# horizon-research/Fov-3DGS

Measured on AMD Instinct MI355X. Metric: frames/sec at 1080p foveated (bicycle-scale), higher is better.
Workload: dtype f32; 1 GPU; S-6M bicycle-scale cloud, 4-layer foveated render (fov_pcheck_obb), the reference's 9 fixed gazes (0.25 i, 0.25 j) in turn, one camera per GPU; gaussians=6000000, width=1920, height=1080, sh_degree=3, model_layout=the reference's tensor interface (render(packed=None)), overlap_successive_frames=True, parallelism=views1

## Files before the change

### fov-3dgs_amd/csrc/common.h

```cpp
#pragma once
#include <hip/hip_runtime.h>
#include <stdint.h>
#include <stddef.h>
#include "../../include/fovraster.h"

#define FR_TILE 16
#define FR_TILE_PIX 256
#define FR_FOV_LEVELS 4
#define FR_FOV_MAX_LEVELS 8
#define FR_SORT_LDS_MAX 8192
#ifndef FR_BIN_THREADS
#define FR_BIN_THREADS 768
#endif
#define FR_BIN_BLOCKS 512
#define FR_PROJ_MAX_WAVES 8192
#define FR_CROW_PAD (64 * FR_PROJ_MAX_WAVES)
#define FR_LDS_HIST_MAX_TILES 16384
#define FR_ITEM_NONE 0xffffffffu
#define FR_LDS_HIST16_MAX_TILES 34816
#define FR_HIST16_MAX_SLABS (65535 / FR_BIN_THREADS)
#define FR_BIG_TNUM 64
#define FR_GIANT_TNUM 1024
#define FR_GIANT_MAX 64
#define FR_SORT_SPLIT_MIN 16384
#define FR_SORT_CHUNK_TARGET 960
#define FR_SORT_FINE_BUCKETS 2048
#define FR_SORT_MAX_CHUNKS(D) ((size_t)(D) / FR_SORT_CHUNK_TARGET + (size_t)(D) / FR_SORT_SPLIT_MIN + 16)
#define FR_LV_BBOX_STRIDE 32
#define FR_SLAB_CTR_WORDS 32

namespace fr {

#define FR_VARIANT_SUM_NOSTATS 100
#define FR_VARIANT_FOV8 101
__host__ __device__ inline bool has_stats(int v) { return v == FR_VARIANT_PCHECK_OBB_SUM || v == FR_VARIANT_PCHECK_OBB_MAX || v == FR_VARIANT_PCHECK_OBB_LWMC; }
__host__ __device__ inline bool has_backward(int v) { return v == FR_VARIANT_ORIGINAL || has_stats(v); }
__host__ __device__ constexpr inline bool is_fov(int v) { return v == FR_VARIANT_FOV_PCHECK_OBB || v == FR_VARIANT_FOV8 || v == FR_VARIANT_NAIVE_FOV_PCHECK_OBB || v == FR_VARIANT_MMFR_PCHECK_OBB; }
// ... 289 lines not shown
{
	const bwd_u2 r = __builtin_amdgcn_permlane16_swap(__float_as_uint(a), __float_as_uint(b), false, false);
	return __uint_as_float(r.x) + __uint_as_float(r.y);
}
__device__ __forceinline__ float row_sum16(float x)
{
	x += __builtin_bit_cast(float, __builtin_amdgcn_update_dpp(0, __builtin_bit_cast(int, x), 0xB1, 0xF, 0xF, false));
	x += __builtin_bit_cast(float, __builtin_amdgcn_update_dpp(0, __builtin_bit_cast(int, x), 0x4E, 0xF, 0xF, false));
	x += __builtin_bit_cast(float, __builtin_amdgcn_update_dpp(0, __builtin_bit_cast(int, x), 0x141, 0xF, 0xF, false));
	x += __builtin_bit_cast(float, __builtin_amdgcn_update_dpp(0, __builtin_bit_cast(int, x), 0x140, 0xF, 0xF, false));
	return x;
}

__device__ __forceinline__ float act_scale(float raw) { return expf(raw); }
__device__ __forceinline__ float act_opacity(float raw) { return 1.0f / (1.0f + expf(-raw)); }
__device__ __forceinline__ float4 act_rotation(float4 v, float *inv_norm = nullptr)
{
	const float n = sqrtf(v.x * v.x + v.y * v.y + v.z * v.z + v.w * v.w);
	const float d = fmaxf(n, 1e-12f);
	if (inv_norm) *inv_norm = n > 1e-12f ? 1.0f / n : -1e12f;
	return make_float4(v.x / d, v.y / d, v.z / d, v.w / d);
}

struct FwdCtx {
	fr_forward_args *a;
	hipStream_t stream;
	int gx, gy, T;
	int fov_split;
	uint8_t *visibility;
	int bin_wgs;
	int hist_mode;
	int scan_fused;
	int heavy4, heavy2;
	int heavy8;
	int heavy16, heavy32;
	int n_items;
	int proj_waves, proj_cpw;
	int64_t capacity;
	int64_t items_cap;
	uint32_t *totals_host_dev;
	uint32_t totals_seq;
	float focal_x, focal_y;
	FovParams fov;
	GeomWS geom;
	ImageWS img;
	BinWS bin;
};
struct AuxStream { int device = -1; hipStream_t main = nullptr, s, s2; hipEvent_t fork, fork2, join, join2; bool ok = false; };
AuxStream *aux_stream(hipStream_t main);
int launch_tile_levels(FwdCtx &c);
int launch_pad_levels(FwdCtx &c);
int launch_pack_geom(int P, const float *means3D, const float *scales, const float *rotations, const float *opacities, int levels,
	const float *highest_levels, float *out, hipStream_t stream);
// ... 34 lines not shown
```

### fov-3dgs_amd/csrc/preprocess.hip

```cpp
#include "common.h"
#include "tile_scan.h"
#include <cstdlib>

namespace fr {

struct M3 { float c[3][3]; };
__device__ __forceinline__ M3 m3_cols(float a0, float a1, float a2, float b0, float b1, float b2, float c0, float c1, float c2)
{
	M3 m; m.c[0][0] = a0; m.c[0][1] = a1; m.c[0][2] = a2; m.c[1][0] = b0; m.c[1][1] = b1; m.c[1][2] = b2;
	m.c[2][0] = c0; m.c[2][1] = c1; m.c[2][2] = c2; return m;
}
__device__ __forceinline__ M3 m3_mul(const M3 &a, const M3 &b)
{
	M3 r;
#pragma unroll
	for (int col = 0; col < 3; col++)
#pragma unroll
		for (int row = 0; row < 3; row++)
			r.c[col][row] = a.c[0][row] * b.c[col][0] + a.c[1][row] * b.c[col][1] + a.c[2][row] * b.c[col][2];
	return r;
}
__device__ __forceinline__ M3 m3_t(const M3 &a)
{
	M3 r;
// ... 828 lines not shown
			const float dch[12] = { dh0.x, dh0.y, dh0.z, dh0.w, dh1.x, dh1.y, dh1.z, dh1.w, dh2.x, dh2.y, dh2.z, dh2.w };
			const float oh[4] = { oph.x, oph.y, oph.z, oph.w };
#pragma unroll
			for (int l = FR_FOV_LEVELS; l < NLV; l++)
			{
				if (l >= lo && l <= hi)
				{
					const int m = l - FR_FOV_LEVELS;
					float4 v;
					v.x = fmaxf(FR_SH_C0 * dch[3 * m] + rest[0], 0.0f);
					v.y = fmaxf(FR_SH_C0 * dch[3 * m + 1] + rest[1], 0.0f);
					v.z = fmaxf(FR_SH_C0 * dch[3 * m + 2] + rest[2], 0.0f);
					v.w = oh[m];
					lv[l] = v;
				}
			}
		}
	}
}

#define BUMP_TILE(ti) do { if (LDSH == 2) atomicAdd(&lds_hist[(ti) >> 1], 1u << (16 * ((ti) & 1))); \
	else if (LDSH) atomicAdd(&lds_hist[(ti)], 1u); else atomicAdd(&a.tile_count[(ti)], 1u); } while (0)
static_assert((FR_BIN_THREADS / 64) * FR_HIST16_MAX_SLABS * 64 <= 65535, "a workgroup's items must fit a 16-bit tile count (LDSH == 2)");
template <int VARIANT, int LDSH, bool PACKED = false, bool CROW = false>
__global__ void __launch_bounds__(FR_BIN_THREADS) k_bin(const PreArgs a)
{
	static_assert(!(PACKED && CROW), "the packed model layout has its own rows");
	constexpr bool CULL = VARIANT != FR_VARIANT_ORIGINAL;
	constexpr bool FOV = is_fov(VARIANT);
	constexpr bool LEVELCOL = is_levelcol(VARIANT);
	constexpr int NLV = level_rows(VARIANT);
	constexpr uint32_t LV_MASK = (1u << NLV) - 1u, LV_BLEND = 1u << NLV;
	static_assert(!(PACKED && FOV && !LEVELCOL), "the shared-model foveated variant has no packed layout");
		extern __shared__ __attribute__((aligned(16))) uint32_t lds_hist[];
	const int lane = threadIdx.x & 63;
	const int hist_words = LDSH == 2 ? (a.T + 1) / 2 : (LDSH ? a.T : 0);
	uint32_t *lds_tab = lds_hist + hist_words;
	const int tab_words = (a.T + 7) / 8;
	const bool ldst = FOV && a.lds_tiles && a.geom.slab_ctr[3] == 0u;
	if (FOV && a.lds_tiles)
	{
		const float *gmin = a.tile_lv + a.T, *gbl = a.tile_lv + 4 * (size_t)a.T;
		for (int t0 = threadIdx.x; t0 < a.T; t0 += 16 * FR_BIN_THREADS)
		{
			float v[16], f[16];
#pragma unroll
			for (int k = 0; k < 16; k++) { const int t = min(t0 + k * FR_BIN_THREADS, a.T - 1); v[k] = gmin[t]; f[k] = gbl[t]; }
#pragma unroll
			for (int k = 0; k < 16; k++)
			{
				const int t = t0 + k * FR_BIN_THREADS;
				uint32_t nib = t < a.T ? ((v[k] == v[k] ? (uint32_t)min(max(f2i(v[k]), 0), 7) : 7u) | (f[k] != 0.0f ? 8u : 0u)) : 0u;
				nib <<= 4 * (lane & 7);
				nib |= (uint32_t)__shfl_xor((int)nib, 1); nib |= (uint32_t)__shfl_xor((int)nib, 2); nib |= (uint32_t)__shfl_xor((int)nib, 4);
				if ((lane & 7) == 0 && (t >> 3) < tab_words) lds_tab[t >> 3] = nib;
			}
		}
	}
	if (LDSH)
		for (int t = threadIdx.x; t < hist_words; t += FR_BIN_THREADS) lds_hist[t] = 0;
	__shared__ int s_gitem[FR_GIANT_MAX];
	__shared__ uint32_t s_gcount[FR_GIANT_MAX], s_gmask[FR_GIANT_MAX];
	__shared__ uint32_t s_ng;
	__shared__ uint4 s_lvbox[5];
	if (FOV && threadIdx.x < 5) s_lvbox[threadIdx.x] = *(const uint4 *)(a.lv_bbox + threadIdx.x * FR_LV_BBOX_STRIDE);
	if (threadIdx.x < FR_GIANT_MAX) { s_gcount[threadIdx.x] = 0; s_gmask[threadIdx.x] = 0; }
	__shared__ uint32_t s_next_slab;
	if (threadIdx.x == 0) { s_ng = 0; s_next_slab = 0; }
	__syncthreads();
#define TILE_FILTER(ti, olim, pass_out, bits_out) do { \
		if (ldst) { const uint32_t nb_ = (lds_tab[(ti) >> 3] >> (4 * ((ti) & 7))) & 15u; \
			pass_out = (float)(nb_ & 7u) < (olim); bits_out = (1u << min(nb_ & 7u, 3u)) | (((nb_ & 8u) >> 3) << NLV); } \
		else { const float lv_ = tile_min[(ti)]; pass_out = lv_ < (olim); \
			bits_out = pass_out ? ((1u << min(max(f2i(lv_), 0), NLV - 1)) | (tile_bl[(ti)] != 0.0f ? LV_BLEND : 0u)) : 0u; } } while (0)
	float4 *const s_orec = (float4 *)(lds_hist + ((hist_words + ((FOV && a.lds_tiles) ? tab_words : 0) + 3) & ~3));
	int *const s_own = (int *)(s_orec + 4 * FR_BIN_THREADS);
	const uint32_t *const s_wbase = (const uint32_t *)(s_own + FR_BIN_THREADS);
	const uint32_t *const g_wbase = a.geom.wbase;
	if (a.wbase_lds)
	{
		uint32_t *const dst = (uint32_t *)(s_own + FR_BIN_THREADS);
		for (int w0 = threadIdx.x; w0 <= a.proj_waves; w0 += 16 * FR_BIN_THREADS)
		{
			uint32_t v[16];
#pragma unroll
			for (int k = 0; k < 16; k++) v[k] = a.geom.wbase[min(w0 + k * FR_BIN_THREADS, a.proj_waves)];
#pragma unroll
			for (int k = 0; k < 16; k++) if (w0 + k * FR_BIN_THREADS <= a.proj_waves) dst[w0 + k * FR_BIN_THREADS] = v[k];
		}
		__syncthreads();
	}
	float cam_vm[16], cam_pm[16];
	{
#pragma unroll
		for (int i = 0; i < 16; i++)
		{
			cam_vm[i] = __builtin_bit_cast(float, __builtin_amdgcn_readfirstlane(__builtin_bit_cast(int, a.viewmatrix[i])));
			cam_pm[i] = __builtin_bit_cast(float, __builtin_amdgcn_readfirstlane(__builtin_bit_cast(int, a.projmatrix[i])));
		}
	}
	const int V = (int)a.geom.slab_ctr[1];
	const int nslabs = (V + 63) / 64;
	const int nwaves = (int)gridDim.x * (FR_BIN_THREADS / 64);
	const float *tile_min = FOV ? a.tile_lv + a.T : nullptr;
	const float *tile_bl = FOV ? a.tile_lv + 4 * (size_t)a.T : nullptr;
	auto walk_uniform = [&](const int ox0, const int oy0, const int ow, const uint32_t on, const Obb &ob, const float olim,
		const uint32_t k0, const uint32_t kstep, uint32_t &cnt, uint32_t &bits) __attribute__((always_inline))
	{
		const float rw = 1.0f / (float)ow;
		for (uint32_t k = k0; k < on; k += kstep)
		{
			const uint32_t j = k + lane;
			const bool valid = j < on;
			int ry = (int)(((float)j + 0.5f) * rw);
			int rx = (int)j - ry * ow;
			if (rx < 0) { ry--; rx += ow; } else if (rx >= ow) { ry++; rx -= ow; }
			const int x = ox0 + rx, y = oy0 + ry;
			const int ti = valid ? y * a.gx + x : 0;
			bool pass = valid;
			uint32_t m = 0;
			if (CULL)
			{
				uint32_t lb = 0;
				if (FOV) { bool lp; TILE_FILTER(ti, olim, lp, lb); pass = pass && lp; }
				pass = pass && obb_hits_tile(ob, x, y);
				if (FOV && pass) m = lb;
// ... 12 lines not shown
	{
		const int lo_bit = __ffs((int)(lvmask & LV_MASK)) - 1, hi_bit = 31 - __clz((int)(lvmask & LV_MASK));
		lowest = fminf(lowest, (float)lo_bit);
		highest = fmaxf(highest, (float)hi_bit);
		be_blend = (lvmask & LV_BLEND) != 0;
	};
	auto range_word = [&](const uint32_t count, const float lowest, const float highest, const bool be_blend) __attribute__((always_inline))
	{
		if (count == 0) return FR_ITEM_NONE;
		if (!FOV) return 0u;
		const int lo = f2i(lowest);
		int hi = f2i(highest);
		if (be_blend) hi = min(hi + 1, a.levels - 1);
		return (uint32_t)(lo & 0xff) | ((uint32_t)(hi & 0xff) << 8);
	};
	float4 *const orec = s_orec + 4 * (threadIdx.x & ~63);
	const bool rows_ok = a.colors_precomp == nullptr &&
		(PACKED || (LEVELCOL ? a.M * 3 >= 45 : (a.shs_rest != nullptr ? (a.M - 1) * 3 >= 45 : a.M * 3 >= 48)));
	for (;;)
	{
	uint32_t q_ = 0;
	if (lane == 0) q_ = atomicAdd(&s_next_slab, 1u);
	q_ = (uint32_t)__builtin_amdgcn_readfirstlane((int)q_);
	constexpr int BW_ = FR_BIN_THREADS / 64;
	const int slab = (int)blockIdx.x * BW_ + (int)(q_ % BW_) + (int)(q_ / BW_) * nwaves;
	if (slab >= nslabs) break;
	const int nv = min(64, V - slab * 64);
	const int item = slab * 64 + lane;
	float4 wr[4];
	float3 fpos = make_float3(0.f, 0.f, 0.f), fconic = make_float3(0.f, 0.f, 0.f);
	{
		RawGaussian g;
		g.p[0] = g.p[1] = g.p[2] = 0.f; g.sc[0] = g.sc[1] = g.sc[2] = 0.f; g.q = make_float4(0, 0, 0, 0); g.hl = 0.f;
		int gidx = 0;
		const bool valid = item < V;
		if (valid)
		{
			auto slot_in = [&](const uint32_t *wb) -> uint32_t {
				int lo = 0, hi = a.proj_waves;
				const uint32_t first = (uint32_t)slab * 64u;
				while (hi - lo > 1) { const int mid = (lo + hi) >> 1; if (wb[mid] <= first) lo = mid; else hi = mid; }
				int w = lo;
				while ((uint32_t)item >= wb[w + 1]) w++;
				return (uint32_t)w * (uint32_t)a.proj_cpw * 64u + ((uint32_t)item - wb[w]);
			};
			const uint32_t slot = a.wbase_lds ? slot_in(s_wbase) : slot_in(g_wbase);
			if (CROW)
// ... 167 lines not shown
#pragma unroll
		for (int l = 0; l < NLV; l++) lv[l] = make_float4(0, 0, 0, 0);
		if (lr != FR_ITEM_NONE) colour_item<VARIANT, PACKED>(a, rows_ok, lr, r, lv);
		if constexpr (LEVELCOL && NLV == FR_FOV_LEVELS) rows_store<4>(lv, orec, a.geom.lvl + 4 * (size_t)slab * 64, nv, lane);
		else if constexpr (LEVELCOL)
		{
			const float4 lo4[4] = { lv[0], lv[1], lv[2], lv[3] }, hi4[4] = { lv[4], lv[5], lv[6], lv[7] };
			rows_store<4>(lo4, orec, a.geom.lvl + 4 * (size_t)slab * 64, nv, lane);
			rows_store<4>(hi4, orec, a.geom.lvl_hi + 4 * (size_t)slab * 64, nv, lane);
		}
		else rows_store<3>(r, orec, a.geom.rec + 3 * (size_t)slab * 64, nv, lane);
	}
	}
	__syncthreads();
	const int ng = min((int)s_ng, FR_GIANT_MAX);
	for (int g = 0; g < ng; g++)
	{
		const float4 *wr = a.geom.wrec + 4 * (size_t)s_gitem[g];
		const float4 w0 = wr[0], w1 = wr[1], w2 = wr[2], w3 = wr[3];
		const Obb ob = make_obb(w0.x, w0.y, make_float4(w0.z, w0.w, w1.x, w1.y), make_float2(w1.z, w1.w));
		const uint32_t xy = __float_as_uint(w2.z);
		uint32_t cnt = 0, bits = 0;
		walk_uniform((int)(xy & 0xffffu), (int)(xy >> 16), (int)__float_as_uint(w2.w), __float_as_uint(w3.x), ob, w3.y + 1,
			(uint32_t)(threadIdx.x & ~63u), (uint32_t)FR_BIN_THREADS, cnt, bits);
		if (lane == 0) { atomicAdd(&s_gcount[g], cnt); if (FOV) atomicOr(&s_gmask[g], bits); }
	}
	__syncthreads();
	if ((int)threadIdx.x < ng)
	{
		const int gitem = s_gitem[threadIdx.x];
		const uint32_t gcount = s_gcount[threadIdx.x];
		const float4 w2 = a.geom.wrec[4 * (size_t)gitem + 2], w3 = a.geom.wrec[4 * (size_t)gitem + 3];
		float lowest = w3.y, highest = 0.0f;
		bool be_blend = false;
		if (FOV && gcount != 0) range_from_mask(s_gmask[threadIdx.x], lowest, highest, be_blend);
		const uint32_t lr = range_word(gcount, lowest, highest, be_blend);
		a.geom.lrange[gitem] = lr;
		if (gcount == 0)
		{
			const uint32_t gi = __float_as_uint(w2.x) & 0x3fffffffu;
			a.radii[gi] = 0;
			if (a.visibility) a.visibility[gi] = 0;
		}
		else
		{
			float4 r[3], lv[NLV];
#pragma unroll
			for (int i = 0; i < 3; i++) r[i] = a.geom.rec[3 * (size_t)gitem + i];
#pragma unroll
			for (int l = 0; l < NLV; l++) lv[l] = make_float4(0, 0, 0, 0);
			colour_item<VARIANT, PACKED>(a, rows_ok, lr, r, lv);
			if (LEVELCOL)
			{
#pragma unroll
				for (int l = 0; l < NLV; l++)
					(l < FR_FOV_LEVELS ? a.geom.lvl : a.geom.lvl_hi)[(size_t)gitem * FR_FOV_LEVELS + (l & 3)] = lv[l];
			}
			else { a.geom.rec[3 * (size_t)gitem + 1] = r[1]; a.geom.rec[3 * (size_t)gitem + 2] = r[2]; }
		}
	}
	if (LDSH)
	{
		__syncthreads();
		uint32_t *out = a.hist + (size_t)blockIdx.x * a.T;
		for (int t0 = threadIdx.x; t0 < a.T; t0 += 4 * FR_BIN_THREADS)
		{
			uint32_t h[4], o[4];
#pragma unroll
			for (int k = 0; k < 4; k++)
			{
				const int t = t0 + k * FR_BIN_THREADS;
				h[k] = t < a.T ? (LDSH == 2 ? (lds_hist[t >> 1] >> (16 * (t & 1))) & 0xffffu : lds_hist[t]) : 0u;
			}
#pragma unroll
			for (int k = 0; k < 4; k++) o[k] = h[k] ? atomicAdd(&a.tile_count[t0 + k * FR_BIN_THREADS], h[k]) : 0u;
#pragma unroll
			for (int k = 0; k < 4; k++) { const int t = t0 + k * FR_BIN_THREADS; if (t < a.T && h[k]) out[t] = o[k]; }
		}
		if (LDSH == 1 && a.fuse_scan)
		{
			__shared__ uint32_t s_last_wg;
			__syncthreads();
			if (threadIdx.x == 0) s_last_wg = atomicAdd(a.geom.slab_ctr + 4, 1u) == gridDim.x - 1 ? 1u : 0u;
			__syncthreads();
			if (!s_last_wg || threadIdx.x >= FR_TILE_SCAN_THREADS) return;
			tile_scan_body<FR_TILE_SCAN_THREADS, true>(a.ts, lds_hist);
		}
	}
}
#undef BUMP_TILE
#undef TILE_FILTER

struct EmitArgs {
	int P, gx, gy, T;
	const int *radii;
	GeomWS geom;
	const float *highest_levels;
	const float *tile_lv;
	const uint32_t *lv_bbox;
	int lds_tiles;
	const uint2 *ranges;
	uint32_t *cursor;
	uint64_t *entries;
	const uint32_t *hist;
	const uint32_t *totals;
	uint32_t capacity;
	uint32_t items_cap;
};
#ifndef FR_EMIT_THREADS
#define FR_EMIT_THREADS FR_BIN_THREADS
#endif
#define NEXT_SLOT(ti) (LDSH == 2 ? a.ranges[(ti)].x + pre_row[(ti)] + ((atomicAdd(&lds_cur[(ti) >> 1], 1u << (16 * ((ti) & 1))) >> (16 * ((ti) & 1))) & 0xffffu) \
	: LDSH ? atomicAdd(&lds_cur[(ti)], 1u) : a.ranges[(ti)].x + atomicAdd(&a.cursor[(ti)], 1u))
template <int VARIANT, int LDSH>
__global__ void __launch_bounds__(FR_EMIT_THREADS) k_emit(const EmitArgs a)
{
	constexpr bool CULL = VARIANT != FR_VARIANT_ORIGINAL;
	constexpr bool FOV = VARIANT == FR_VARIANT_FOV_PCHECK_OBB;
	extern __shared__ __attribute__((aligned(16))) uint32_t lds_cur[];
#ifdef FR_EMIT_TIMERS
	const uint64_t tm_entry = wall_clock64(); uint64_t tm_pro = 0, tm_loop = 0, tm_walk = 0, tm_big = 0, tm_drain = 0, tm_pre = 0, tm_mid = 0, tm_ta = 0; int tm_slabs = 0, tm_steps = 0;
#endif
	if (a.totals[0] > a.capacity || a.totals[5] > a.items_cap) return;
	const int lane = threadIdx.x & 63;
	const int cur_words = LDSH == 2 ? (a.T + 1) / 2 : (LDSH ? a.T : 0);
	const uint32_t *const pre_row = a.hist + (LDSH ? (size_t)blockIdx.x * a.T : 0);
	uint32_t *lds_tab = lds_cur + cur_words;
	const int tab_words = (a.T + 7) / 8;
	const bool ldst = FOV && a.lds_tiles && a.geom.slab_ctr[3] == 0u;
	if (ldst)
// ... 172 lines not shown
					const float xp = tpx + 8.0f - o0.x, xm = tpx - 8.0f - o0.x, yp = tpy + 8.0f - o0.y, ym = tpy - 8.0f - o0.y;
					const float a1p = xp * o0.z, a1m = xm * o0.z, b1p = yp * o0.w, b1m = ym * o0.w;
					const float mn1 = fminf(a1p, a1m) + fminf(b1p, b1m), mx1 = fmaxf(a1p, a1m) + fmaxf(b1p, b1m);
					const bool e1_ok = !(o1.z < mn1 || -o1.z > mx1);
					const float a2p = xp * o1.x, a2m = xm * o1.x, b2p = yp * o1.y, b2m = ym * o1.y;
					const float mn2 = fminf(a2p, a2m) + fminf(b2p, b2m), mx2 = fmaxf(a2p, a2m) + fmaxf(b2p, b2m);
					const bool e2_ok = !(o1.w < mn2 || -o1.w > mx2);
					pass = pass && cx_ok && cy_ok && e1_ok && e2_ok;
				}
			}
			if (pass) a.entries[NEXT_SLOT(ti)] = opay;
		}
		if (total != 0)
		{
			__builtin_amdgcn_fence(__ATOMIC_RELEASE, "wavefront");
			__builtin_amdgcn_wave_barrier();
		}
#ifdef FR_EMIT_TIMERS
		tm_walk += wall_clock64() - tw0;
#endif
	}
	};
	{
		constexpr int BW = FR_BIN_THREADS / 64;
		const int bin_waves = (int)gridDim.x * BW;
		auto slab_of = [&](const int s) { return (int)blockIdx.x * BW + s % BW + (s / BW) * bin_waves; };
		auto grab = [&]() -> int {
			uint32_t q_ = 0;
			if (lane == 0) q_ = atomicAdd(&s_next_slab, 1u);
			return slab_of(__builtin_amdgcn_readfirstlane((int)q_));
		};
		SlabIn cur, nxt;
		int slab = grab();
		if (slab < nslabs) fetch_slab(slab, cur);
#ifdef FR_EMIT_TIMERS
		const uint64_t tl0 = wall_clock64();
#endif
		for (; slab < nslabs; )
		{
#ifdef FR_EMIT_TIMERS
			tm_ta = wall_clock64();
#endif
			const int next = grab();
			const bool more = next < nslabs;
			if (more) fetch_slab(next, nxt);
			process(slab, cur);
#ifdef FR_EMIT_TIMERS
// ... 145 lines not shown
	p.tanfovx = a->tanfovx; p.tanfovy = a->tanfovy; p.focal_x = c.focal_x; p.focal_y = c.focal_y;
	p.scale_modifier = a->scale_modifier;
	p.means3D = a->means3D; p.scales = a->scales; p.rotations = a->rotations; p.opacities = a->opacities;
	p.shs = a->shs; p.shs_rest = a->shs_rest; p.cov3D_precomp = a->cov3D_precomp; p.colors_precomp = a->colors_precomp;
	p.viewmatrix = a->viewmatrix; p.projmatrix = a->projmatrix; p.campos = a->campos;
	p.packed_geom = a->packed_geom; p.packed_colour = a->packed_colour; p.packed_cull = a->packed_cull;
	p.shs_dcs = a->shs_dcs; p.highest_levels = a->highest_levels; p.tile_lv = c.img.tile_lv; p.lv_bbox = c.img.lv_bbox; p.T = c.T;
	p.levels = c.fov.levels;
	if (c.geom.pad_op != nullptr && !a->packed_geom) { p.opacities = c.geom.pad_op; p.shs_dcs = c.geom.pad_dc; }
	p.radii = a->radii; p.visibility = c.visibility; p.clear_color = c.fov_split ? a->out_color : nullptr; p.geom = c.geom; p.tile_count = c.img.tile_count; p.hist = c.img.hist; p.raw = a->raw_activations;
	p.write_cov3D = has_backward(a->variant) ? 1 : 0;
	p.prefiltered = a->prefiltered;
	p.proj_waves = c.proj_waves; p.proj_cpw = c.proj_cpw;
	p.fuse_scan = 0;
	return p;
}

int launch_project(FwdCtx &c)
{
	const fr_forward_args *a = c.a;
	PreArgs p = make_pre_args(c);
	{
		static thread_local int resident_of[8][6];
		int cur_dev = 0;
		(void)hipGetDevice(&cur_dev);
		int *const resident = resident_of[cur_dev & 7];
		const bool packed = a->packed_cull != nullptr;
		const int vslot = a->variant == FR_VARIANT_ORIGINAL ? 0 : (is_fov(a->variant) ? 1 : 2);
		const int slot = vslot + (packed ? 3 : 0);
		if (resident[slot] == 0)
		{
			int per_cu = 0, dev = 0;
			hipDeviceProp_t prop;
			const void *fns[6] = { (const void *)k_project<FR_VARIANT_ORIGINAL>, (const void *)k_project<FR_VARIANT_FOV_PCHECK_OBB>,
				(const void *)k_project<FR_VARIANT_PCHECK_OBB>, (const void *)k_project<FR_VARIANT_ORIGINAL, true>,
				(const void *)k_project<FR_VARIANT_FOV_PCHECK_OBB, true>, (const void *)k_project<FR_VARIANT_PCHECK_OBB, true> };
			const void *fn = fns[slot];
			if (hipGetDevice(&dev) != hipSuccess || hipGetDeviceProperties(&prop, dev) != hipSuccess ||
				hipOccupancyMaxActiveBlocksPerMultiprocessor(&per_cu, fn, FR_PROJ_THREADS, 0) != hipSuccess || per_cu < 1)
			{ per_cu = 4; prop.multiProcessorCount = 256; }
			resident[slot] = per_cu * prop.multiProcessorCount;
		}
		const int pchunks = (a->P + FR_PROJ_THREADS - 1) / FR_PROJ_THREADS;
		const int pmax = resident[slot] < FR_PROJ_MAX_WAVES / (FR_PROJ_THREADS / 64) ? resident[slot] : FR_PROJ_MAX_WAVES / (FR_PROJ_THREADS / 64);
		const dim3 pgrid(pchunks < pmax ? pchunks : pmax), pblock(FR_PROJ_THREADS);
		c.proj_waves = (int)pgrid.x * (FR_PROJ_THREADS / 64);
		c.proj_cpw = proj_chunks_per_wave(a->P, c.proj_waves);
		p.proj_waves = c.proj_waves; p.proj_cpw = c.proj_cpw;
#define LAUNCH_PROJ(V) do { if (packed) hipLaunchKernelGGL((k_project<V, true>), pgrid, pblock, 0, c.stream, p); \
	else hipLaunchKernelGGL((k_project<V>), pgrid, pblock, 0, c.stream, p); } while (0)
		switch (vslot)
		{
		case 0: LAUNCH_PROJ(FR_VARIANT_ORIGINAL); break;
		case 1: LAUNCH_PROJ(FR_VARIANT_FOV_PCHECK_OBB); break;
		default: LAUNCH_PROJ(FR_VARIANT_PCHECK_OBB); break;
		}
#undef LAUNCH_PROJ
		return check_launch("project", c.stream, a->debug);
	}
}

int launch_bin(FwdCtx &c)
{
	const fr_forward_args *a = c.a;
	PreArgs p = make_pre_args(c);
	int nblk = bin_blocks(a->P);
	const dim3 block(FR_BIN_THREADS);
	static thread_local int cus = 0;
	if (cus == 0)
	{
		int dev = 0; hipDeviceProp_t prop;
		cus = (hipGetDevice(&dev) == hipSuccess && hipGetDeviceProperties(&prop, dev) == hipSuccess && prop.multiProcessorCount > 0) ? prop.multiProcessorCount : 64;
		(void)hipGetLastError();
	}
	const int64_t wgs_lo = nblk < cus ? nblk : cus;
	c.hist_mode = c.img.hist == nullptr ? 0 : (c.T <= FR_LDS_HIST_MAX_TILES ? 1 :
		(wgs_lo * (FR_BIN_THREADS / 64) * (int64_t)(FR_HIST16_MAX_SLABS - 1) * 64 >= (int64_t)a->P ? 2 : 0));
	const bool ldsh = c.hist_mode != 0;
	p.lds_tiles = (is_fov(a->variant) && ldsh) ? 1 : 0;
	const size_t hist_bytes = c.hist_mode == 2 ? (size_t)((c.T + 1) / 2) * sizeof(uint32_t) : (ldsh ? (size_t)c.T * sizeof(uint32_t) : 0);
	const size_t lds_fixed = ((hist_bytes + (p.lds_tiles ? lds_tile_table_bytes(c.T) : 0) + 15) & ~(size_t)15) +
		(size_t)FR_BIN_THREADS * (4 * sizeof(float4) + sizeof(int));
	const size_t wbase_bytes = (size_t)(c.proj_waves + 1) * sizeof(uint32_t);
	p.wbase_lds = lds_fixed + wbase_bytes <= 156u * 1024u ? 1 : 0;
	size_t lds = lds_fixed + (p.wbase_lds ? wbase_bytes : 0);
	static const bool fuse_ok = []() { const char *e = getenv("FOVRASTER_FUSE_SCAN"); return !(e && e[0] == '0'); }();
	c.scan_fused = fuse_ok && c.hist_mode == 1 && c.T <= FR_SCAN_MAX_TILES && !a->debug;
	if (c.scan_fused)
	{
		p.fuse_scan = 1; p.ts = make_tile_scan_args(c);
		const size_t scan_bytes = (size_t)tile_scan_lds_words<FR_TILE_SCAN_THREADS>() * sizeof(uint32_t);
		if (lds < scan_bytes) lds = scan_bytes;
	}
	auto launch = [&](const void *fn, void (*kern)(const PreArgs), size_t dyn) {
		static thread_local struct { const void *fn; size_t dyn; int wgs; } cache[48];
		static thread_local int ncache = 0;
		int wgs = 0;
		for (int i = 0; i < ncache; i++) if (cache[i].fn == fn && cache[i].dyn == dyn) wgs = cache[i].wgs;
		if (wgs == 0)
		{
			if (dyn > 64u * 1024u && hipFuncSetAttribute(fn, hipFuncAttributeMaxDynamicSharedMemorySize, (int)dyn) != hipSuccess)
			{ set_error("hipFuncSetAttribute(k_bin): %s", hipGetErrorString(hipGetLastError())); return FR_ERR_HIP; }
			int per_cu = 0, dev = 0;
			hipDeviceProp_t prop;
			if (hipGetDevice(&dev) != hipSuccess || hipGetDeviceProperties(&prop, dev) != hipSuccess ||
				hipOccupancyMaxActiveBlocksPerMultiprocessor(&per_cu, fn, FR_BIN_THREADS, dyn) != hipSuccess || per_cu < 1)
			{ per_cu = 1; prop.multiProcessorCount = 256; (void)hipGetLastError(); }
			wgs = per_cu * prop.multiProcessorCount;
			if (ncache < 48) { cache[ncache].fn = fn; cache[ncache].dyn = dyn; cache[ncache].wgs = wgs; ncache++; }
		}
		nblk = nblk < wgs ? nblk : wgs;
		hipLaunchKernelGGL(kern, dim3(nblk), block, dyn, c.stream, p);
		return FR_OK;
	};
	int lrc = FR_OK;
	const bool packed = a->packed_geom && a->packed_colour;
	const bool crow = !packed && is_fov(a->variant) && a->packed_cull == nullptr && a->cov3D_precomp == nullptr;
#define LAUNCH_BIN_PC(V, PK, CR) do { if (c.hist_mode == 2) lrc = launch((const void *)k_bin<V, 2, PK, CR>, k_bin<V, 2, PK, CR>, lds); \
	else if (ldsh) lrc = launch((const void *)k_bin<V, 1, PK, CR>, k_bin<V, 1, PK, CR>, lds); \
	else lrc = launch((const void *)k_bin<V, 0, PK, CR>, k_bin<V, 0, PK, CR>, lds); } while (0)
#define LAUNCH_BIN(V) do { if (packed) LAUNCH_BIN_PC(V, true, false); else if (crow) LAUNCH_BIN_PC(V, false, true); else LAUNCH_BIN_PC(V, false, false); } while (0)
	switch (a->variant)
	{
	case FR_VARIANT_ORIGINAL: LAUNCH_BIN(FR_VARIANT_ORIGINAL); break;
	case FR_VARIANT_FOV_PCHECK_OBB:
		if (c.fov.levels <= FR_FOV_LEVELS) LAUNCH_BIN(FR_VARIANT_FOV_PCHECK_OBB);
		else if (crow) LAUNCH_BIN_PC(FR_VARIANT_FOV8, false, true);
		else LAUNCH_BIN_PC(FR_VARIANT_FOV8, false, false);
		break;
	case FR_VARIANT_MMFR_PCHECK_OBB:
	case FR_VARIANT_NAIVE_FOV_PCHECK_OBB:
		if (crow) LAUNCH_BIN_PC(FR_VARIANT_NAIVE_FOV_PCHECK_OBB, false, true); else LAUNCH_BIN_PC(FR_VARIANT_NAIVE_FOV_PCHECK_OBB, false, false);
		break;
	default: LAUNCH_BIN(FR_VARIANT_PCHECK_OBB); break;
	}
#undef LAUNCH_BIN
#undef LAUNCH_BIN_PC
	if (lrc) return lrc;
	c.bin_wgs = nblk;
	return check_launch("bin", c.stream, a->debug);
}

int launch_emit(FwdCtx &c)
{
	const fr_forward_args *a = c.a;
	EmitArgs e;
	e.P = a->P; e.gx = c.gx; e.gy = c.gy; e.T = c.T; e.radii = a->radii; e.geom = c.geom;
	e.highest_levels = a->highest_levels; e.tile_lv = c.img.tile_lv; e.lv_bbox = c.img.lv_bbox; e.ranges = c.img.ranges;
	e.cursor = c.img.tile_count; e.entries = c.bin.entries; e.hist = c.img.hist;
	e.totals = c.img.totals; e.capacity = (uint32_t)c.capacity; e.items_cap = (uint32_t)c.items_cap;
	const bool ldsh = c.hist_mode != 0;
	const dim3 grid(c.bin_wgs), block(FR_EMIT_THREADS);
	e.lds_tiles = (is_fov(a->variant) && ldsh) ? 1 : 0;
	const size_t lds = (((c.hist_mode == 2 ? (size_t)((c.T + 1) / 2) * sizeof(uint32_t) : (ldsh ? (size_t)c.T * sizeof(uint32_t) : 0)) +
		(e.lds_tiles ? lds_tile_table_bytes(c.T) : 0) + 15) & ~(size_t)15) + (size_t)FR_EMIT_THREADS * 4 * sizeof(float4);
	if (lds > 64u * 1024u)
	{
		static const hipError_t once = []() {
			const void *fns[] = { (const void *)k_emit<FR_VARIANT_ORIGINAL, 0>, (const void *)k_emit<FR_VARIANT_ORIGINAL, 1>, (const void *)k_emit<FR_VARIANT_ORIGINAL, 2>,
				(const void *)k_emit<FR_VARIANT_PCHECK_OBB, 0>, (const void *)k_emit<FR_VARIANT_PCHECK_OBB, 1>, (const void *)k_emit<FR_VARIANT_PCHECK_OBB, 2>,
				(const void *)k_emit<FR_VARIANT_FOV_PCHECK_OBB, 0>, (const void *)k_emit<FR_VARIANT_FOV_PCHECK_OBB, 1>, (const void *)k_emit<FR_VARIANT_FOV_PCHECK_OBB, 2> };
			for (const void *fn : fns)
			{
				const hipError_t e1 = hipFuncSetAttribute(fn, hipFuncAttributeMaxDynamicSharedMemorySize, (FR_EMIT_THREADS > 768 ? 154 : 156) * 1024);
				if (e1 != hipSuccess) return e1;
			}
			return hipSuccess; }();
		if (once != hipSuccess) { set_error("hipFuncSetAttribute(k_emit): %s", hipGetErrorString(once)); return FR_ERR_HIP; }
	}
#define LAUNCH_EMIT(V) do { if (c.hist_mode == 2) hipLaunchKernelGGL((k_emit<V, 2>), grid, block, lds, c.stream, e); \
	else if (ldsh) hipLaunchKernelGGL((k_emit<V, 1>), grid, block, lds, c.stream, e); \
	else hipLaunchKernelGGL((k_emit<V, 0>), grid, block, lds, c.stream, e); } while (0)
	switch (a->variant)
// ... 19 lines not shown
```

### fov-3dgs_amd/rasterizer.py

```python
import contextlib
import ctypes as C
import os
import threading
import time
from typing import NamedTuple

import torch
import torch.nn as nn

from . import _native


class GaussianRasterizationSettings(NamedTuple):
    image_height: int
    image_width: int
    tanfovx: float
    tanfovy: float
    bg: torch.Tensor
    scale_modifier: float
    viewmatrix: torch.Tensor
    projmatrix: torch.Tensor
    sh_degree: int
    campos: torch.Tensor
    prefiltered: bool
# ... 396 lines not shown
        a.out_color, a.radii = color.data_ptr(), radii.data_ptr()
        put("loss_map", loss_map)
        if list_consumed is not None:
            tiles = ((W + 15) // 16) * ((H + 15) // 16)
            if list_consumed.device != dev or list_consumed.numel() != tiles or list_consumed.element_size() != 4 or not list_consumed.is_contiguous():
                raise RuntimeError(f"list_consumed must be a contiguous 4-byte integer tensor of {tiles} tiles on {dev}")
            keep.append(list_consumed)
            a.list_consumed = list_consumed.data_ptr()
        if blend_pairs is not None:
            tiles = ((W + 15) // 16) * ((H + 15) // 16)
            if blend_pairs.device != dev or blend_pairs.numel() != tiles or blend_pairs.element_size() != 4 or not blend_pairs.is_contiguous():
                raise RuntimeError(f"blend_pairs must be a contiguous 4-byte integer tensor of {tiles} tiles on {dev}")
            keep.append(blend_pairs)
            a.blend_pairs = blend_pairs.data_ptr()
        if packed is not None:
            packed.check(P, dev)
            if packed.produced is not None:
                packed.produced.wait_on_current(dev)
            a.packed_geom = _ptr(packed.geom)
            a.packed_colour = _ptr(packed.colour)
            a.packed_cull = _ptr(packed.cull)
            keep.append(packed)
        a.no_stats = int(bool(no_stats))
        a.no_helper_streams = int(persistent and INFERENCE_NO_HELPER_STREAMS)
        if variant in (_native.VARIANT_PCHECK_OBB_SUM, _native.VARIANT_PCHECK_OBB_MAX, _native.VARIANT_PCHECK_OBB_LWMC) and not no_stats:
            counts = torch.empty((P,), dtype=torch.int32, device=dev)
            contribs = torch.empty((P,), dtype=torch.float32, device=dev)
            a.gaussians_count, a.contributions = counts.data_ptr(), contribs.data_ptr()
        a.geometry_resize, a.binning_resize, a.image_resize = ws.cbs[0], ws.cbs[1], ws.cbs[2]
        if _stage_events_hook is not None:
            a.stage_events = _stage_events_hook()
        handle = C.c_void_p()
        rc = _begin_call(lib, a, P, dev, radii, handle, fov)
        if rc != 0:
            raise RuntimeError(f"fovraster forward failed ({rc}): {_native.last_error()}")
    if reuse is not None:
        reuse.clear()
        if reuse_key is not None and counts is None and lease is None:
            reuse.update(key=reuse_key, a=a, keep=own, ws=ws, fov=fov)
    return FrameInFlight(lib, a, keep, color, radii, ws, lease, counts, contribs, handle, dev, stream)


OVERLAP_SUCCESSIVE_FRAMES = os.environ.get("FOVRASTER_OVERLAP", "1") != "0"
_overlap_state = {}
_overlap_tls = threading.local()


# ... 697 lines not shown
```

### include/fovraster.h

```cpp
#ifndef FOVRASTER_H
#define FOVRASTER_H

#include <stddef.h>
#include <stdint.h>

#ifdef __cplusplus
extern "C" {
#endif

#define FR_ABI_VERSION 12

enum {
	FR_VARIANT_ORIGINAL = 0,
	FR_VARIANT_PCHECK_OBB_SUM = 1,
	FR_VARIANT_PCHECK_OBB = 2,
	FR_VARIANT_FOV_PCHECK_OBB = 3,
	FR_VARIANT_PCHECK_OBB_MAX = 4,
	FR_VARIANT_PCHECK_OBB_LWMC = 5,
	FR_VARIANT_NAIVE_FOV_PCHECK_OBB = 6,
	FR_VARIANT_MMFR_PCHECK_OBB = 7
};

enum {
	FR_OK = 0,
// ... 36 lines not shown
	int32_t *gaussians_count;
	float *contributions;
	fr_resize_fn geometry_resize;
	fr_resize_fn binning_resize;
	fr_resize_fn image_resize;
	void *resize_user[3];
	int32_t num_rendered;
	int32_t max_tile_instances;
	void **stage_events;
	const float *loss_map;
	const float *shs_rest;
	const float *packed_geom;
	const float *packed_colour;
	const float *packed_cull;
	float cur_level;
	int32_t raw_activations;
	int32_t num_candidates;
	uint32_t *list_consumed;
	int32_t no_stats;
	uint32_t *blend_pairs;
	int32_t no_helper_streams;
} fr_forward_args;

enum { FR_STAGE_TILE_LEVELS = 0, FR_STAGE_PROJECT = 1, FR_STAGE_BIN = 2, FR_STAGE_TILE_SCAN = 3, FR_STAGE_EMIT = 4,
	FR_STAGE_TILE_SORT = 5, FR_STAGE_RENDER = 6, FR_NUM_STAGES = 7 };

typedef struct fr_backward_args {
	int32_t variant;
	int32_t P, D, M, R;
	int32_t W, H;
	int32_t debug;
	float tanfovx, tanfovy;
	float scale_modifier;
	void *stream;
	const float *background, *means3D, *shs, *colors_precomp, *opacities, *scales, *rotations,
		*cov3D_precomp, *viewmatrix, *projmatrix, *campos;
	const int32_t *radii;
	char *geometry;
	const char *binning, *image;
	const float *dL_dpix;
	float *dL_dmean2D;
	float *dL_dconic;
	float *dL_dopacity;
	float *dL_dcolor;
	float *dL_dmean3D;
	float *dL_dcov3D;
// ... 247 lines not shown
```

Baseline: 2242 frames/s.

## Shrink projection grid and bin workgroups when successive frames share the GPU

Adds a flag, set when persistent frames reuse state, that marks a frame as sharing the GPU with an overlapping frame. When it is set, the projection grid is capped at a fraction of the CU count, and the foveated binning kernel runs with smaller workgroups through a new thread-count template parameter. The emit kernel now reads the bin wave count at runtime. The aim is to leave room for the overlapping frame's kernels to co-run rather than one frame's stages taking every CU. The risk is lower single-frame throughput in those stages if the overlap does not actually fill the freed CUs.

```diff
diff --git a/fov-3dgs_amd/csrc/common.h b/fov-3dgs_amd/csrc/common.h
--- a/fov-3dgs_amd/csrc/common.h
+++ b/fov-3dgs_amd/csrc/common.h
@@ -2,6 +2,7 @@
 #include <hip/hip_runtime.h>
 #include <stdint.h>
 #include <stddef.h>
+#include <stdlib.h>
 #include "../../include/fovraster.h"
 
 #define FR_TILE 16
@@ -13,6 +14,13 @@
 #define FR_BIN_THREADS 768
 #endif
 #define FR_BIN_BLOCKS 512
+#ifndef FR_PROJ_SHARED_NUM
+#define FR_PROJ_SHARED_NUM 3
+#define FR_PROJ_SHARED_DEN 4
+#endif
+#ifndef FR_BIN_SHARED_THREADS
+#define FR_BIN_SHARED_THREADS 512
+#endif
 #define FR_PROJ_MAX_WAVES 8192
 #define FR_CROW_PAD (64 * FR_PROJ_MAX_WAVES)
 #define FR_LDS_HIST_MAX_TILES 16384
@@ -348,6 +356,12 @@
 	return make_float4(v.x / d, v.y / d, v.z / d, v.w / d);
 }
 
+inline bool frame_shares_gpu(const fr_forward_args *a)
+{
+	static const bool lone = []() { const char *e = getenv("FOVRASTER_LONE_GEOMETRY"); return e && e[0] == '1'; }();
+	return (a->no_helper_streams & FR_FRAME_SHARES_GPU) != 0 && !lone;
+}
+
 struct FwdCtx {
 	fr_forward_args *a;
 	hipStream_t stream;
@@ -355,6 +369,7 @@
 	int fov_split;
 	uint8_t *visibility;
 	int bin_wgs;
+	int bin_bw;
 	int hist_mode;
 	int scan_fused;
 	int heavy4, heavy2;
diff --git a/fov-3dgs_amd/csrc/preprocess.hip b/fov-3dgs_amd/csrc/preprocess.hip
--- a/fov-3dgs_amd/csrc/preprocess.hip
+++ b/fov-3dgs_amd/csrc/preprocess.hip
@@ -874,9 +874,11 @@
 #define BUMP_TILE(ti) do { if (LDSH == 2) atomicAdd(&lds_hist[(ti) >> 1], 1u << (16 * ((ti) & 1))); \
 	else if (LDSH) atomicAdd(&lds_hist[(ti)], 1u); else atomicAdd(&a.tile_count[(ti)], 1u); } while (0)
 static_assert((FR_BIN_THREADS / 64) * FR_HIST16_MAX_SLABS * 64 <= 65535, "a workgroup's items must fit a 16-bit tile count (LDSH == 2)");
-template <int VARIANT, int LDSH, bool PACKED = false, bool CROW = false>
-__global__ void __launch_bounds__(FR_BIN_THREADS) k_bin(const PreArgs a)
-{
+template <int VARIANT, int LDSH, bool PACKED = false, bool CROW = false, int BT = FR_BIN_THREADS>
+__global__ void __launch_bounds__(BT) k_bin(const PreArgs a)
+{
+	static_assert(BT % 64 == 0 && BT >= FR_TILE_SCAN_THREADS && (LDSH != 2 || (BT / 64) * FR_HIST16_MAX_SLABS * 64 <= 65535),
+		"whole waves, enough of them for the fused tile scan, and (LDSH == 2) a workgroup's items within a 16-bit tile count");
 	static_assert(!(PACKED && CROW), "the packed model layout has its own rows");
 	constexpr bool CULL = VARIANT != FR_VARIANT_ORIGINAL;
 	constexpr bool FOV = is_fov(VARIANT);
@@ -893,15 +895,15 @@
 	if (FOV && a.lds_tiles)
 	{
 		const float *gmin = a.tile_lv + a.T, *gbl = a.tile_lv + 4 * (size_t)a.T;
-		for (int t0 = threadIdx.x; t0 < a.T; t0 += 16 * FR_BIN_THREADS)
+		for (int t0 = threadIdx.x; t0 < a.T; t0 += 16 * BT)
 		{
 			float v[16], f[16];
 #pragma unroll
-			for (int k = 0; k < 16; k++) { const int t = min(t0 + k * FR_BIN_THREADS, a.T - 1); v[k] = gmin[t]; f[k] = gbl[t]; }
+			for (int k = 0; k < 16; k++) { const int t = min(t0 + k * BT, a.T - 1); v[k] = gmin[t]; f[k] = gbl[t]; }
 #pragma unroll
 			for (int k = 0; k < 16; k++)
 			{
-				const int t = t0 + k * FR_BIN_THREADS;
+				const int t = t0 + k * BT;
 				uint32_t nib = t < a.T ? ((v[k] == v[k] ? (uint32_t)min(max(f2i(v[k]), 0), 7) : 7u) | (f[k] != 0.0f ? 8u : 0u)) : 0u;
 				nib <<= 4 * (lane & 7);
 				nib |= (uint32_t)__shfl_xor((int)nib, 1); nib |= (uint32_t)__shfl_xor((int)nib, 2); nib |= (uint32_t)__shfl_xor((int)nib, 4);
@@ -910,7 +912,7 @@
 		}
 	}
 	if (LDSH)
-		for (int t = threadIdx.x; t < hist_words; t += FR_BIN_THREADS) lds_hist[t] = 0;
+		for (int t = threadIdx.x; t < hist_words; t += BT) lds_hist[t] = 0;
 	__shared__ int s_gitem[FR_GIANT_MAX];
 	__shared__ uint32_t s_gcount[FR_GIANT_MAX], s_gmask[FR_GIANT_MAX];
 	__shared__ uint32_t s_ng;
@@ -926,19 +928,19 @@
 		else { const float lv_ = tile_min[(ti)]; pass_out = lv_ < (olim); \
 			bits_out = pass_out ? ((1u << min(max(f2i(lv_), 0), NLV - 1)) | (tile_bl[(ti)] != 0.0f ? LV_BLEND : 0u)) : 0u; } } while (0)
 	float4 *const s_orec = (float4 *)(lds_hist + ((hist_words + ((FOV && a.lds_tiles) ? tab_words : 0) + 3) & ~3));
-	int *const s_own = (int *)(s_orec + 4 * FR_BIN_THREADS);
-	const uint32_t *const s_wbase = (const uint32_t *)(s_own + FR_BIN_THREADS);
+	int *const s_own = (int *)(s_orec + 4 * BT);
+	const uint32_t *const s_wbase = (const uint32_t *)(s_own + BT);
 	const uint32_t *const g_wbase = a.geom.wbase;
 	if (a.wbase_lds)
 	{
-		uint32_t *const dst = (uint32_t *)(s_own + FR_BIN_THREADS);
-		for (int w0 = threadIdx.x; w0 <= a.proj_waves; w0 += 16 * FR_BIN_THREADS)
+		uint32_t *const dst = (uint32_t *)(s_own + BT);
+		for (int w0 = threadIdx.x; w0 <= a.proj_waves; w0 += 16 * BT)
 		{
 			uint32_t v[16];
 #pragma unroll
-			for (int k = 0; k < 16; k++) v[k] = a.geom.wbase[min(w0 + k * FR_BIN_THREADS, a.proj_waves)];
-#pragma unroll
-			for (int k = 0; k < 16; k++) if (w0 + k * FR_BIN_THREADS <= a.proj_waves) dst[w0 + k * FR_BIN_THREADS] = v[k];
+			for (int k = 0; k < 16; k++) v[k] = a.geom.wbase[min(w0 + k * BT, a.proj_waves)];
+#pragma unroll
+			for (int k = 0; k < 16; k++) if (w0 + k * BT <= a.proj_waves) dst[w0 + k * BT] = v[k];
 		}
 		__syncthreads();
 	}
@@ -953,7 +955,7 @@
 	}
 	const int V = (int)a.geom.slab_ctr[1];
 	const int nslabs = (V + 63) / 64;
-	const int nwaves = (int)gridDim.x * (FR_BIN_THREADS / 64);
+	const int nwaves = (int)gridDim.x * (BT / 64);
 	const float *tile_min = FOV ? a.tile_lv + a.T : nullptr;
 	const float *tile_bl = FOV ? a.tile_lv + 4 * (size_t)a.T : nullptr;
 	auto walk_uniform = [&](const int ox0, const int oy0, const int ow, const uint32_t on, const Obb &ob, const float olim,
@@ -1012,7 +1014,7 @@
 	uint32_t q_ = 0;
 	if (lane == 0) q_ = atomicAdd(&s_next_slab, 1u);
 	q_ = (uint32_t)__builtin_amdgcn_readfirstlane((int)q_);
-	constexpr int BW_ = FR_BIN_THREADS / 64;
+	constexpr int BW_ = BT / 64;
 	const int slab = (int)blockIdx.x * BW_ + (int)(q_ % BW_) + (int)(q_ / BW_) * nwaves;
 	if (slab >= nslabs) break;
 	const int nv = min(64, V - slab * 64);
@@ -1226,7 +1228,7 @@
 		const uint32_t xy = __float_as_uint(w2.z);
 		uint32_t cnt = 0, bits = 0;
 		walk_uniform((int)(xy & 0xffffu), (int)(xy >> 16), (int)__float_as_uint(w2.w), __float_as_uint(w3.x), ob, w3.y + 1,
-			(uint32_t)(threadIdx.x & ~63u), (uint32_t)FR_BIN_THREADS, cnt, bits);
+			(uint32_t)(threadIdx.x & ~63u), (uint32_t)BT, cnt, bits);
 		if (lane == 0) { atomicAdd(&s_gcount[g], cnt); if (FOV) atomicOr(&s_gmask[g], bits); }
 	}
 	__syncthreads();
@@ -1267,19 +1269,19 @@
 	{
 		__syncthreads();
 		uint32_t *out = a.hist + (size_t)blockIdx.x * a.T;
-		for (int t0 = threadIdx.x; t0 < a.T; t0 += 4 * FR_BIN_THREADS)
+		for (int t0 = threadIdx.x; t0 < a.T; t0 += 4 * BT)
 		{
 			uint32_t h[4], o[4];
 #pragma unroll
 			for (int k = 0; k < 4; k++)
 			{
-				const int t = t0 + k * FR_BIN_THREADS;
+				const int t = t0 + k * BT;
 				h[k] = t < a.T ? (LDSH == 2 ? (lds_hist[t >> 1] >> (16 * (t & 1))) & 0xffffu : lds_hist[t]) : 0u;
 			}
 #pragma unroll
-			for (int k = 0; k < 4; k++) o[k] = h[k] ? atomicAdd(&a.tile_count[t0 + k * FR_BIN_THREADS], h[k]) : 0u;
-#pragma unroll
-			for (int k = 0; k < 4; k++) { const int t = t0 + k * FR_BIN_THREADS; if (t < a.T && h[k]) out[t] = o[k]; }
+			for (int k = 0; k < 4; k++) o[k] = h[k] ? atomicAdd(&a.tile_count[t0 + k * BT], h[k]) : 0u;
+#pragma unroll
+			for (int k = 0; k < 4; k++) { const int t = t0 + k * BT; if (t < a.T && h[k]) out[t] = o[k]; }
 		}
 		if (LDSH == 1 && a.fuse_scan)
 		{
@@ -1310,6 +1312,7 @@
 	const uint32_t *totals;
 	uint32_t capacity;
 	uint32_t items_cap;
+	int bin_bw;
 };
 #ifndef FR_EMIT_THREADS
 #define FR_EMIT_THREADS FR_BIN_THREADS
@@ -1528,7 +1531,7 @@
 	}
 	};
 	{
-		constexpr int BW = FR_BIN_THREADS / 64;
+		const int BW = a.bin_bw;
 		const int bin_waves = (int)gridDim.x * BW;
 		auto slab_of = [&](const int s) { return (int)blockIdx.x * BW + s % BW + (s / BW) * bin_waves; };
 		auto grab = [&]() -> int {
@@ -1720,6 +1723,7 @@
 	PreArgs p = make_pre_args(c);
 	{
 		static thread_local int resident_of[8][6];
+		static thread_local int cus_of[8];
 		int cur_dev = 0;
 		(void)hipGetDevice(&cur_dev);
 		int *const resident = resident_of[cur_dev & 7];
@@ -1738,9 +1742,13 @@
 				hipOccupancyMaxActiveBlocksPerMultiprocessor(&per_cu, fn, FR_PROJ_THREADS, 0) != hipSuccess || per_cu < 1)
 			{ per_cu = 4; prop.multiProcessorCount = 256; }
 			resident[slot] = per_cu * prop.multiProcessorCount;
-		}
+			cus_of[cur_dev & 7] = prop.multiProcessorCount;
+		}
+		const bool shared = frame_shares_gpu(a);
+		int cap = resident[slot];
+		if (shared) { const int part = (int)((int64_t)cus_of[cur_dev & 7] * FR_PROJ_SHARED_NUM / FR_PROJ_SHARED_DEN); cap = part < cap ? (part > 0 ? part : 1) : cap; }
 		const int pchunks = (a->P + FR_PROJ_THREADS - 1) / FR_PROJ_THREADS;
-		const int pmax = resident[slot] < FR_PROJ_MAX_WAVES / (FR_PROJ_THREADS / 64) ? resident[slot] : FR_PROJ_MAX_WAVES / (FR_PROJ_THREADS / 64);
+		const int pmax = cap < FR_PROJ_MAX_WAVES / (FR_PROJ_THREADS / 64) ? cap : FR_PROJ_MAX_WAVES / (FR_PROJ_THREADS / 64);
 		const dim3 pgrid(pchunks < pmax ? pchunks : pmax), pblock(FR_PROJ_THREADS);
 		c.proj_waves = (int)pgrid.x * (FR_PROJ_THREADS / 64);
 		c.proj_cpw = proj_chunks_per_wave(a->P, c.proj_waves);
@@ -1763,7 +1771,6 @@
 	const fr_forward_args *a = c.a;
 	PreArgs p = make_pre_args(c);
 	int nblk = bin_blocks(a->P);
-	const dim3 block(FR_BIN_THREADS);
 	static thread_local int cus = 0;
 	if (cus == 0)
 	{
@@ -1775,10 +1782,16 @@
 	c.hist_mode = c.img.hist == nullptr ? 0 : (c.T <= FR_LDS_HIST_MAX_TILES ? 1 :
 		(wgs_lo * (FR_BIN_THREADS / 64) * (int64_t)(FR_HIST16_MAX_SLABS - 1) * 64 >= (int64_t)a->P ? 2 : 0));
 	const bool ldsh = c.hist_mode != 0;
+	const bool packed = a->packed_geom && a->packed_colour;
+	const bool crow = !packed && is_fov(a->variant) && a->packed_cull == nullptr && a->cov3D_precomp == nullptr;
+	const bool shared = FR_BIN_SHARED_THREADS != FR_BIN_THREADS && frame_shares_gpu(a) && a->variant == FR_VARIANT_FOV_PCHECK_OBB &&
+		c.fov.levels <= FR_FOV_LEVELS && c.hist_mode == 1 && (packed || crow);
+	const int bt = shared ? FR_BIN_SHARED_THREADS : FR_BIN_THREADS;
+	const dim3 block(bt);
 	p.lds_tiles = (is_fov(a->variant) && ldsh) ? 1 : 0;
 	const size_t hist_bytes = c.hist_mode == 2 ? (size_t)((c.T + 1) / 2) * sizeof(uint32_t) : (ldsh ? (size_t)c.T * sizeof(uint32_t) : 0);
 	const size_t lds_fixed = ((hist_bytes + (p.lds_tiles ? lds_tile_table_bytes(c.T) : 0) + 15) & ~(size_t)15) +
-		(size_t)FR_BIN_THREADS * (4 * sizeof(float4) + sizeof(int));
+		(size_t)bt * (4 * sizeof(float4) + sizeof(int));
 	const size_t wbase_bytes = (size_t)(c.proj_waves + 1) * sizeof(uint32_t);
 	p.wbase_lds = lds_fixed + wbase_bytes <= 156u * 1024u ? 1 : 0;
 	size_t lds = lds_fixed + (p.wbase_lds ? wbase_bytes : 0);
@@ -1802,7 +1815,7 @@
 			int per_cu = 0, dev = 0;
 			hipDeviceProp_t prop;
 			if (hipGetDevice(&dev) != hipSuccess || hipGetDeviceProperties(&prop, dev) != hipSuccess ||
-				hipOccupancyMaxActiveBlocksPerMultiprocessor(&per_cu, fn, FR_BIN_THREADS, dyn) != hipSuccess || per_cu < 1)
+				hipOccupancyMaxActiveBlocksPerMultiprocessor(&per_cu, fn, bt, dyn) != hipSuccess || per_cu < 1)
 			{ per_cu = 1; prop.multiProcessorCount = 256; (void)hipGetLastError(); }
 			wgs = per_cu * prop.multiProcessorCount;
 			if (ncache < 48) { cache[ncache].fn = fn; cache[ncache].dyn = dyn; cache[ncache].wgs = wgs; ncache++; }
@@ -1812,8 +1825,6 @@
 		return FR_OK;
 	};
 	int lrc = FR_OK;
-	const bool packed = a->packed_geom && a->packed_colour;
-	const bool crow = !packed && is_fov(a->variant) && a->packed_cull == nullptr && a->cov3D_precomp == nullptr;
 #define LAUNCH_BIN_PC(V, PK, CR) do { if (c.hist_mode == 2) lrc = launch((const void *)k_bin<V, 2, PK, CR>, k_bin<V, 2, PK, CR>, lds); \
 	else if (ldsh) lrc = launch((const void *)k_bin<V, 1, PK, CR>, k_bin<V, 1, PK, CR>, lds); \
 	else lrc = launch((const void *)k_bin<V, 0, PK, CR>, k_bin<V, 0, PK, CR>, lds); } while (0)
@@ -1822,7 +1833,14 @@
 	{
 	case FR_VARIANT_ORIGINAL: LAUNCH_BIN(FR_VARIANT_ORIGINAL); break;
 	case FR_VARIANT_FOV_PCHECK_OBB:
-		if (c.fov.levels <= FR_FOV_LEVELS) LAUNCH_BIN(FR_VARIANT_FOV_PCHECK_OBB);
+		if (shared)
+		{
+			if (packed) lrc = launch((const void *)k_bin<FR_VARIANT_FOV_PCHECK_OBB, 1, true, false, FR_BIN_SHARED_THREADS>,
+				k_bin<FR_VARIANT_FOV_PCHECK_OBB, 1, true, false, FR_BIN_SHARED_THREADS>, lds);
+			else lrc = launch((const void *)k_bin<FR_VARIANT_FOV_PCHECK_OBB, 1, false, true, FR_BIN_SHARED_THREADS>,
+				k_bin<FR_VARIANT_FOV_PCHECK_OBB, 1, false, true, FR_BIN_SHARED_THREADS>, lds);
+		}
+		else if (c.fov.levels <= FR_FOV_LEVELS) LAUNCH_BIN(FR_VARIANT_FOV_PCHECK_OBB);
 		else if (crow) LAUNCH_BIN_PC(FR_VARIANT_FOV8, false, true);
 		else LAUNCH_BIN_PC(FR_VARIANT_FOV8, false, false);
 		break;
@@ -1835,7 +1853,7 @@
 #undef LAUNCH_BIN
 #undef LAUNCH_BIN_PC
 	if (lrc) return lrc;
-	c.bin_wgs = nblk;
+	c.bin_wgs = nblk; c.bin_bw = bt / 64;
 	return check_launch("bin", c.stream, a->debug);
 }
 
@@ -1846,7 +1864,7 @@
 	e.P = a->P; e.gx = c.gx; e.gy = c.gy; e.T = c.T; e.radii = a->radii; e.geom = c.geom;
 	e.highest_levels = a->highest_levels; e.tile_lv = c.img.tile_lv; e.lv_bbox = c.img.lv_bbox; e.ranges = c.img.ranges;
 	e.cursor = c.img.tile_count; e.entries = c.bin.entries; e.hist = c.img.hist;
-	e.totals = c.img.totals; e.capacity = (uint32_t)c.capacity; e.items_cap = (uint32_t)c.items_cap;
+	e.totals = c.img.totals; e.capacity = (uint32_t)c.capacity; e.items_cap = (uint32_t)c.items_cap; e.bin_bw = c.bin_bw;
 	const bool ldsh = c.hist_mode != 0;
 	const dim3 grid(c.bin_wgs), block(FR_EMIT_THREADS);
 	e.lds_tiles = (is_fov(a->variant) && ldsh) ? 1 : 0;
diff --git a/fov-3dgs_amd/rasterizer.py b/fov-3dgs_amd/rasterizer.py
--- a/fov-3dgs_amd/rasterizer.py
+++ b/fov-3dgs_amd/rasterizer.py
@@ -442,7 +442,7 @@
             a.packed_cull = _ptr(packed.cull)
             keep.append(packed)
         a.no_stats = int(bool(no_stats))
-        a.no_helper_streams = int(persistent and INFERENCE_NO_HELPER_STREAMS)
+        a.no_helper_streams = int(persistent and INFERENCE_NO_HELPER_STREAMS) * (3 if reuse is not None else 1)
         if variant in (_native.VARIANT_PCHECK_OBB_SUM, _native.VARIANT_PCHECK_OBB_MAX, _native.VARIANT_PCHECK_OBB_LWMC) and not no_stats:
             counts = torch.empty((P,), dtype=torch.int32, device=dev)
             contribs = torch.empty((P,), dtype=torch.float32, device=dev)
diff --git a/include/fovraster.h b/include/fovraster.h
--- a/include/fovraster.h
+++ b/include/fovraster.h
@@ -82,6 +82,8 @@
 	int32_t no_helper_streams;
 } fr_forward_args;
 
+enum { FR_FRAME_NO_HELPER_STREAMS = 1, FR_FRAME_SHARES_GPU = 2 };
+
 enum { FR_STAGE_TILE_LEVELS = 0, FR_STAGE_PROJECT = 1, FR_STAGE_BIN = 2, FR_STAGE_TILE_SCAN = 3, FR_STAGE_EMIT = 4,
 	FR_STAGE_TILE_SORT = 5, FR_STAGE_RENDER = 6, FR_NUM_STAGES = 7 };
 
```

Result: faster. 2423 frames/s (median of 6 runs) (+8.1%).
